# chen-bowen/instacart_next_order_recommendation

Hardware: AMD Instinct MI355X
Metric: recommend_qps_top20_49k7_catalog (higher is better)
Workload: dtype f16x3 (f32 operands split into 2 f16 planes, 3 f16 MFMAs per product, f32 accumulate; fp32-level accuracy)

## Files before the change

### instacart_next_order_recommendation_amd/csrc/encoder.hip

```cpp
#include <stdlib.h>

#include <mutex>
#include <type_traits>
#include <vector>

#include "common.h"
#include "wt_gemm.h"
#include "encoder_x3.h"

namespace icrec {

__device__ __forceinline__ int find_seq(const int32_t* __restrict__ cu, int n_seqs, int t) {
    int lo = 0, hi = n_seqs;
    while (hi - lo > 1) {
        int mid = (lo + hi) >> 1;
        if (cu[mid] <= t) lo = mid; else hi = mid;
    }
    return lo;
}

template <int H, bool SPLIT>
__device__ __forceinline__ void ln_row(float (&v)[H / 64], const float* __restrict__ g, const float* __restrict__ b,
                                       float eps, float* __restrict__ out, _Float16* __restrict__ oh,
                                       _Float16* __restrict__ ol, int lane) {
// ... 134 lines not shown
    const int tid = threadIdx.x, lane = tid & 63, wave = tid >> 6;
    const int s = blockIdx.x / heads, hd = blockIdx.x % heads;
    const int t0 = cu[s], L = cu[s + 1] - t0;
    const int nkt = (L + 31) >> 5;
    if (nkt > NKT || nkt <= nlo) return;
    const int ld = 3 * H;
    const int r = lane & 31, h = lane >> 5, qb = wave;
    const bool active = qb < nkt;
    const float* bt = nullptr;
    if constexpr (BIAS) {
        __shared__ __attribute__((aligned(16))) float Bs[ATT_BIAS_LD];
        att_bias_to_lds(Bs, bias, hd, tid, NKT * 64);
        bt = Bs + att_bias_base(qb, lane);
    }
    float4 qf[D / 8];
    {
        int qr = qb * 32 + r;
        qr = qr < L ? qr : L - 1;
        const float4* qp = reinterpret_cast<const float4*>(qkv + (size_t)(t0 + qr) * ld + hd * D);
#pragma unroll
        for (int kq = 0; kq < D / 8; ++kq) {
            const float4 a = qp[2 * kq], b = qp[2 * kq + 1];
            qf[kq] = h == 0 ? make_float4(a.x, a.z, b.x, b.z) : make_float4(a.y, a.w, b.y, b.w);
        }
    }
    const bool once = KC == NKT || nkt <= KC;
    auto stage = [&](int c0, bool with_v) {
        if (!once) __syncthreads();
        const int nk = (nkt - c0 < KC ? nkt - c0 : KC) * 32;
        for (int id = tid; id < nk * (D / 4); id += NKT * 64) {
            const int row = id / (D / 4), c = id % (D / 4);
            const int key = c0 * 32 + row, rr = key < L ? key : L - 1;
            const float* src = qkv + (size_t)(t0 + rr) * ld + hd * D + c * 4;
            const float4 kv = *reinterpret_cast<const float4*>(src + H);
            float* kp = Ks + row * LDK + (c >> 1) * 8 + (c & 1) * 2;
            *reinterpret_cast<float2*>(kp) = make_float2(kv.x, kv.z);
            *reinterpret_cast<float2*>(kp + 4) = make_float2(kv.y, kv.w);
            if (with_v) *reinterpret_cast<float4*>(Vs + row * D + c * 4) = *reinterpret_cast<const float4*>(src + 2 * H);
        }
        __syncthreads();
    };
    auto score_tile = [&](int kt, int c0) {
        f32x16 t;
#pragma unroll
        for (int e = 0; e < 16; ++e) t[e] = 0.0f;
#pragma unroll
        for (int kq = 0; kq < D / 8; ++kq) {
            const float4 kf = *reinterpret_cast<const float4*>(Ks + ((kt - c0) * 32 + r) * LDK + kq * 8 + h * 4);
            t = __builtin_amdgcn_mfma_f32_32x32x2f32(kf.x, qf[kq].x, t, 0, 0, 0);
            t = __builtin_amdgcn_mfma_f32_32x32x2f32(kf.y, qf[kq].y, t, 0, 0, 0);
            t = __builtin_amdgcn_mfma_f32_32x32x2f32(kf.z, qf[kq].z, t, 0, 0, 0);
            t = __builtin_amdgcn_mfma_f32_32x32x2f32(kf.w, qf[kq].w, t, 0, 0, 0);
        }
        const bool last = kt == nkt - 1;
#pragma unroll
        for (int e = 0; e < 16; ++e) {
            float v;
            if constexpr (BIAS) v = fmaf(t[e], scale_log2e, bt[kt * 32 + (e & 3) + 8 * (e >> 2)]);
            else v = t[e] * scale_log2e;
            if (last && kt * 32 + acc_row(e, lane) >= L) v = -INFINITY;
            t[e] = v;
        }
        return t;
    };
    f32x16 o[D / 32];
#pragma unroll
    for (int dt = 0; dt < D / 32; ++dt)
#pragma unroll
        for (int e = 0; e < 16; ++e) o[dt][e] = 0.0f;
    auto pv_tile = [&](int kt, int c0, const f32x16& p) {
#pragma unroll
        for (int e = 0; e < 16; ++e) {
            const int key = (kt - c0) * 32 + (e & 3) + 8 * (e >> 2) + 4 * h;
#pragma unroll
            for (int dt = 0; dt < D / 32; ++dt)
                o[dt] = __builtin_amdgcn_mfma_f32_32x32x2f32(p[e], Vs[key * D + 32 * dt + r], o[dt], 0, 0, 0);
        }
    };
    auto for_tiles = [&](bool with_v, auto&& f) {
#pragma unroll
        for (int c0 = 0; c0 < NKT; c0 += KC) {
            if (c0 < nkt) {
                if (!once) stage(c0, with_v);
                if (active) {
                    const int c1 = c0 + KC < nkt ? c0 + KC : nkt;
                    for (int kt = c0; kt < c1; ++kt) f(kt, c0);
                }
            }
        }
    };
    if (once) stage(0, true);
    float lsum = 0.0f;
    if constexpr (RECOMP) {
        float mx = -INFINITY;
        for_tiles(false, [&](int kt, int c0) {
            const f32x16 t = score_tile(kt, c0);
#pragma unroll
            for (int e = 0; e < 16; ++e) mx = fmaxf(mx, t[e]);
        });
        mx = fmaxf(mx, __shfl_xor(mx, 32, 64));
        for_tiles(true, [&](int kt, int c0) {
            f32x16 t = score_tile(kt, c0);
#pragma unroll
            for (int e = 0; e < 16; ++e) {
                const float p = __builtin_amdgcn_exp2f(t[e] - mx);
                t[e] = p;
                lsum = lsum + p;
            }
            pv_tile(kt, c0, t);
        });
    } else if (active) {
        f32x16 sc[NKT];
        float mx = -INFINITY;
#pragma unroll
        for (int kt = 0; kt < NKT; ++kt) {
            if (kt < nkt) {
                sc[kt] = score_tile(kt, 0);
#pragma unroll
                for (int e = 0; e < 16; ++e) mx = fmaxf(mx, sc[kt][e]);
            }
        }
        mx = fmaxf(mx, __shfl_xor(mx, 32, 64));
#pragma unroll
        for (int kt = 0; kt < NKT; ++kt) {
            if (kt < nkt) {
#pragma unroll
                for (int e = 0; e < 16; ++e) {
                    const float p = __builtin_amdgcn_exp2f(sc[kt][e] - mx);
                    sc[kt][e] = p;
                    lsum = lsum + p;
                }
            }
        }
#pragma unroll
        for (int kt = 0; kt < NKT; ++kt)
            if (kt < nkt) pv_tile(kt, 0, sc[kt]);
    }
    if (!active) return;
    lsum = join_halves(lsum, h);
    if (h == 0) Ls[wave * 32 + r] = lsum;
#pragma unroll
    for (int e = 0; e < 16; ++e) {
        const int qrow = acc_row(e, lane);
        const int tq = qb * 32 + qrow;
        if (tq < L) {
            const float l = Ls[wave * 32 + qrow];
            float* dst = ctx + (size_t)(t0 + tq) * H + hd * D + r;
#pragma unroll
            for (int dt = 0; dt < D / 32; ++dt) dst[32 * dt] = o[dt][e] / l;
        }
    }
}

__global__ __launch_bounds__(1024) void seq_order_kernel(const int32_t* __restrict__ cu, int n_seqs,
                                                         int32_t* __restrict__ order) {
    constexpr int NB = ICREC_MAX_SEQLEN / 32;
    __shared__ int hist[NB];
    const int tid = threadIdx.x;
    if (tid < NB) hist[tid] = 0;
    __syncthreads();
    auto bin = [&](int s) {
        const int L = cu[s + 1] - cu[s];
        const int nkt = (L + 31) >> 5;
        return NB - (nkt < 1 ? 1 : (nkt > NB ? NB : nkt));
    };
    for (int s0 = tid; s0 < n_seqs; s0 += 1024) atomicAdd(&hist[bin(n_seqs - 1 - s0)], 1);
    __syncthreads();
    if (tid == 0) {
        int run = 0;
        for (int b = 0; b < NB; ++b) { const int c = hist[b]; hist[b] = run; run += c; }
    }
    __syncthreads();
    for (int s0 = tid; s0 < n_seqs; s0 += 1024) {
        const int s = n_seqs - 1 - s0;
        order[atomicAdd(&hist[bin(s)], 1)] = s;
    }
}

typedef _Float16 half2v __attribute__((ext_vector_type(2)));

__device__ __forceinline__ half4 lds_read_tr(const _Float16* p) {
    typedef __fp16 fp16x4 __attribute__((__vector_size__(4 * sizeof(__fp16))));
    return __builtin_bit_cast(half4, __builtin_amdgcn_ds_read_tr16_b64_v4f16(
                                         (__attribute__((address_space(3))) fp16x4*)(reinterpret_cast<uintptr_t>(p))));
}

constexpr int att_k_swz(int D, int row) { return D == 32 ? (row >> 2) & 3 : row & 7; }
constexpr int att_x3_wgs(int D, int NKT) { return D != 32 ? 1 : NKT >= 6 ? 4 : NKT == 4 ? 3 : 1; }

template <int D, int NKT, bool BIAS = false>
__global__ __launch_bounds__(NKT * 64, att_x3_wgs(D, NKT)) void attention_x3_kernel(
    const float* __restrict__ qkv, const int32_t* __restrict__ cu, int heads, int H, float scale_log2e,
    _Float16* __restrict__ ch, _Float16* __restrict__ cl, const int32_t* __restrict__ order, int nlo, int nqb,
    const float* __restrict__ bias) {
    constexpr int KC = att_kc(D, NKT), G = D / 4;
    constexpr bool RECOMP = D == 64 || NKT >= 6;
    constexpr bool PREFETCH = D == 32, PARK = D == 32;
    static_assert(!PARK || KC == NKT, "the parked output tiles need the K planes of all NKT key tiles");
    __shared__ __attribute__((aligned(16))) _Float16 Kbuf[2 * KC * 32 * D];
    _Float16* const Kh = Kbuf;
    _Float16* const Kl = Kbuf + KC * 32 * D;
    __shared__ __attribute__((aligned(16))) _Float16 Vh[KC * 32 * D];
    __shared__ __attribute__((aligned(16))) _Float16 Vl[KC * 32 * D];
    __shared__ float Ls[NKT * 32];

    const int tid = threadIdx.x, lane = tid & 63, wave = tid >> 6;
    const int sidx = blockIdx.x / heads, hd = blockIdx.x % heads;
    const int s = order != nullptr ? order[sidx] : sidx;
    const int t0 = cu[s], L = cu[s + 1] - t0;
    const int nkt = (L + 31) >> 5;
    if (nkt > NKT || nkt <= nlo) return;
    const int ld = 3 * H;
    const int r = lane & 31, h = lane >> 5, qb = wave;
    const bool active = qb < nkt && qb < nqb;
    const float* bt = nullptr;
    if constexpr (BIAS) {
        __shared__ __attribute__((aligned(16))) float Bs[ATT_BIAS_LD];
        att_bias_to_lds(Bs, bias, hd, tid, NKT * 64);
        bt = Bs + att_bias_base(qb, lane);
    }
    half8 qh[D / 16], ql[D / 16];
    {
        int qr = qb * 32 + r;
        qr = qr < L ? qr : L - 1;
        const float* qp = qkv + (size_t)(t0 + qr) * ld + hd * D;
#pragma unroll
        for (int ks = 0; ks < D / 16; ++ks) {
            const f32x4 a = *reinterpret_cast<const f32x4*>(qp + 16 * ks + 8 * h);
            const f32x4 b = *reinterpret_cast<const f32x4*>(qp + 16 * ks + 8 * h + 4);
            half4 ah, al, bh, bl;
            split_act4(a, ah, al);
            split_act4(b, bh, bl);
            qh[ks] = half8{ah[0], ah[1], ah[2], ah[3], bh[0], bh[1], bh[2], bh[3]};
            ql[ks] = half8{al[0], al[1], al[2], al[3], bl[0], bl[1], bl[2], bl[3]};
        }
    }
    const bool once = KC == NKT || nkt <= KC;
    auto stage = [&](int c0, bool with_v) {
        if (!once) __syncthreads();
        const int nk = (nkt - c0 < KC ? nkt - c0 : KC) * 32;
        auto src_of = [&](int id) {
            const int key = c0 * 32 + id / G, rr = key < L ? key : L - 1;
            return qkv + (size_t)(t0 + rr) * ld + hd * D + (id % G) * 4;
        };
        auto put = [&](int id, const f32x4& k, const f32x4& v) {
            const int row = id / G, c = id % G;
            half4 khi, klo;
            split_act4(k, khi, klo);
            if (with_v) {
                half4 vhi, vlo;
                split_act4(v, vhi, vlo);
                *reinterpret_cast<half4*>(Vh + row * D + c * 4) = vhi;
                *reinterpret_cast<half4*>(Vl + row * D + c * 4) = vlo;
            }
            const int off = row * D + ((((c >> 1) ^ att_k_swz(D, row)) << 3) | ((c & 1) << 2));
            *reinterpret_cast<half4*>(Kh + off) = khi;
            *reinterpret_cast<half4*>(Kl + off) = klo;
        };
        if constexpr (PREFETCH) {
            constexpr int STG = KC * 32 * G / (NKT * 64);
            static_assert(KC * 32 * G % (NKT * 64) == 0, "staging: whole rounds");
            f32x4 kreg[STG], vreg[STG];
#pragma unroll
            for (int it = 0; it < STG; ++it) {
                const float* src = src_of(tid + it * NKT * 64);
                kreg[it] = *reinterpret_cast<const f32x4*>(src + H);
                if (with_v) vreg[it] = *reinterpret_cast<const f32x4*>(src + 2 * H);
            }
#pragma unroll
            for (int it = 0; it < STG; ++it)
                if (tid + it * NKT * 64 < nk * G) put(tid + it * NKT * 64, kreg[it], vreg[it]);
        } else {
            for (int id = tid; id < nk * G; id += NKT * 64) {
                const float* src = src_of(id);
                f32x4 v = {0.0f, 0.0f, 0.0f, 0.0f};
                if (with_v) v = *reinterpret_cast<const f32x4*>(src + 2 * H);
                put(id, *reinterpret_cast<const f32x4*>(src + H), v);
            }
        }
        __syncthreads();
    };
    auto score_tile = [&](int kt, int c0, bool hi_only) {
        f32x16 t;
#pragma unroll
        for (int e = 0; e < 16; ++e) t[e] = 0.0f;
        const int row = (kt - c0) * 32 + r;
#pragma unroll
        for (int ks = 0; ks < D / 16; ++ks) {
            const int off = row * D + (((2 * ks + h) ^ att_k_swz(D, row)) << 3);
            const half8 kh = *reinterpret_cast<const half8*>(Kh + off);
            const half8 kl = *reinterpret_cast<const half8*>(Kl + off);
            t = __builtin_amdgcn_mfma_f32_32x32x16_f16(kh, qh[ks], t, 0, 0, 0);
            if (hi_only) continue;
            t = __builtin_amdgcn_mfma_f32_32x32x16_f16(kh, ql[ks], t, 0, 0, 0);
            t = __builtin_amdgcn_mfma_f32_32x32x16_f16(kl, qh[ks], t, 0, 0, 0);
        }
        if (kt == nkt - 1 && kt * 32 + 32 > L) {
#pragma unroll
            for (int e = 0; e < 16; ++e)
                if (kt * 32 + acc_row(e, lane) >= L) t[e] = -INFINITY;
        }
        return t;
    };
    f32x16 o[D / 32];
#pragma unroll
    for (int dt = 0; dt < D / 32; ++dt)
#pragma unroll
        for (int e = 0; e < 16; ++e) o[dt][e] = 0.0f;
    auto pv_tile = [&](int kt, int c0, const f32x16& pt) {
#pragma unroll
        for (int ks = 0; ks < 2; ++ks) {
            half8 ph, pl;
#pragma unroll
            for (int j = 0; j < 8; j += 2) {
                half2w a, b;
                split_pair_prescaled(pt[8 * ks + j], pt[8 * ks + j + 1], a, b);
                ph[j] = a[0]; ph[j + 1] = a[1];
                pl[j] = b[0]; pl[j + 1] = b[1];
            }
            const int base = (kt - c0) * 32 + 4 * h + 16 * ks;
#pragma unroll
            for (int dt = 0; dt < D / 32; ++dt) {
                const int tr_at = (base + ((lane & 15) >> 2)) * D + 32 * dt + 16 * ((lane >> 4) & 1) + 4 * (lane & 3);
                const half4 v0h = lds_read_tr(Vh + tr_at);
                const half4 v1h = lds_read_tr(Vh + tr_at + 8 * D);
                const half4 v0l = lds_read_tr(Vl + tr_at);
                const half4 v1l = lds_read_tr(Vl + tr_at + 8 * D);
                const half8 vh = {v0h[0], v0h[1], v0h[2], v0h[3], v1h[0], v1h[1], v1h[2], v1h[3]};
                const half8 vl = {v0l[0], v0l[1], v0l[2], v0l[3], v1l[0], v1l[1], v1l[2], v1l[3]};
                o[dt] = __builtin_amdgcn_mfma_f32_32x32x16_f16(ph, vh, o[dt], 0, 0, 0);
                o[dt] = __builtin_amdgcn_mfma_f32_32x32x16_f16(ph, vl, o[dt], 0, 0, 0);
                o[dt] = __builtin_amdgcn_mfma_f32_32x32x16_f16(pl, vh, o[dt], 0, 0, 0);
            }
        }
    };
    auto for_tiles = [&](bool with_v, auto&& f) {
#pragma unroll
        for (int c0 = 0; c0 < NKT; c0 += KC) {
            if (c0 < nkt) {
                if (!once) stage(c0, with_v);
                if (active) {
#pragma unroll
                    for (int j = 0; j < KC; ++j)
                        if (c0 + j < nkt) f(c0 + j, c0);
                }
            }
        }
    };
    typedef float float2w __attribute__((ext_vector_type(2)));
    const float cs = scale_log2e * (1.0f / 256.0f);
    auto biased = [&](f32x16& t, int kt) {
#pragma unroll
        for (int e = 0; e < 16; ++e) t[e] = fmaf(t[e], cs, bt[kt * 32 + (e & 3) + 8 * (e >> 2)]);
    };
    float2w ls2 = float2w{0.0f, 0.0f};
    auto join_rows = [&]() {
        const float lrow = join_halves(ls2[0] + ls2[1], h);
        if (h == 0) Ls[wave * 32 + r] = lrow;
    };
    if (once) stage(0, true);
// ... 224 lines not shown
    __syncthreads();
    float* const ps = hs;
#pragma unroll
    for (int r = 0; r < JPT; ++r)
#pragma unroll
        for (int sl = 0; sl < S; ++sl) ps[(tid + 384 * r) * S + sl] = tanhf(acc[r][sl]);
    __syncthreads();
    if (tid < S && s0 + tid < n_seqs) {
        float logit = bc[0];
        for (int j = 0; j < H; ++j) logit = fmaf(wc[j], ps[j * S + tid], logit);
        scores[s0 + tid] = logit;
    }
}

constexpr int HID = 384;
constexpr int HID_BASE = 768;
template <class F>
static auto for_hidden(int hidden, F f) {
    return hidden == HID_BASE ? f(std::integral_constant<int, HID_BASE>{}) : f(std::integral_constant<int, HID>{});
}

struct LayerW {
    float *Wqkv, *bqkv, *Wo, *bo, *g1, *b1n, *W1, *b1, *W2, *b2, *g2, *b2n;
    _Float16 *Wqkv_p, *Wo_p, *W1_p, *W2_p;
};
struct Encoder {
    icrec_bert_cfg cfg;
    int device = 0;
    int n_cu = 256;
    int max_seqlen = 256;
    int pooling = ICREC_POOL_MEAN;
    float* att_bias = nullptr;
    float* score_head = nullptr;
    float* blob = nullptr;
    float* extra = nullptr;
    _Float16* planes = nullptr;
    float *word, *pos, *type, *eg, *eb;
    LayerW layers[64];
    bool fuse = true, side_stream = true, cls_prune = true;
    int small_m = 3584;
    int tail_m = 2560;
    struct Side {
        hipStream_t caller = nullptr, side = nullptr;
        hipEvent_t ev = nullptr;
    };
    std::mutex side_mu;
    std::vector<Side*> sides;
};

static int side_for(Encoder* e, hipStream_t caller, Encoder::Side** out) {
    std::lock_guard<std::mutex> lock(e->side_mu);
    *out = nullptr;
    for (Encoder::Side* sd : e->sides)
        if (sd->caller == caller) { *out = sd; return ICREC_OK; }
    hipStreamCaptureStatus cap = hipStreamCaptureStatusNone;
    if (caller && hipStreamIsCapturing(caller, &cap) == hipSuccess && cap != hipStreamCaptureStatusNone)
        return ICREC_OK;
    Encoder::Side* sd = new Encoder::Side();
    sd->caller = caller;
    ICREC_HIP(hipStreamCreateWithFlags(&sd->side, hipStreamNonBlocking));
    ICREC_HIP(hipEventCreateWithFlags(&sd->ev, hipEventDisableTiming));
    e->sides.push_back(sd);
    *out = sd;
    return ICREC_OK;
}

static size_t weight_count(const icrec_bert_cfg* c) {
    const size_t H = c->hidden, I = c->intermediate;
    const size_t emb = (size_t)c->vocab_size * H + (size_t)c->max_position * H + (size_t)c->type_vocab * H + 2 * H;
    const size_t per = 4 * (H * H + H) + 2 * H + (I * H + I) + (H * I + H) + 2 * H;
    return emb + per * c->layers;
}

struct EncWs {
    size_t x, xs, qkv, ctx, t1, h, total;
};
static EncWs enc_ws(const icrec_bert_cfg& c, int64_t T, bool post_only = false) {
    auto al = [](size_t b) { return (b + 255) & ~(size_t)255; };
    EncWs w;
    size_t o = 0;
    w.x = o;   o += post_only ? 0 : al((size_t)T * c.hidden * 4);
    w.xs = o;  o += al((size_t)T * c.hidden * 4);
    w.qkv = o; o += post_only ? 0 : al((size_t)T * 3 * c.hidden * 4);
    w.ctx = o; o += al((size_t)T * c.hidden * 4);
    w.t1 = o;  o += al((size_t)T * c.hidden * 4);
    w.h = o;   o += al((size_t)T * c.intermediate * 4);
    w.total = o;
    return w;
}

struct EncBufs {
    float *x, *qkv, *ctx, *t1, *h;
    _Float16 *xh, *xl, *ch, *cl, *hh, *hl;
    EncBufs(char* base, const EncWs& w, const icrec_bert_cfg& c, size_t T)
        : x(reinterpret_cast<float*>(base + w.x)), qkv(reinterpret_cast<float*>(base + w.qkv)),
          ctx(reinterpret_cast<float*>(base + w.ctx)), t1(reinterpret_cast<float*>(base + w.t1)),
          h(reinterpret_cast<float*>(base + w.h)), xh(reinterpret_cast<_Float16*>(base + w.xs)), xl(xh + T * c.hidden),
          ch(reinterpret_cast<_Float16*>(ctx)), cl(ch + T * c.hidden), hh(reinterpret_cast<_Float16*>(h)),
          hl(hh + T * c.intermediate) {}
};

static bool cls_prunes(const Encoder* e) {
    return e->pooling == ICREC_POOL_CLS && e->cls_prune && e->cfg.gemm_mode == ICREC_GEMM_F16X3;
}

typedef TileCfg<2, 2, 2, 2> GemmBig;
constexpr long long SMALL_M_MAX = 1 << 20;

static int env_knob(const char* name, int fallback, long long hi) {
    const char* s = getenv(name);
    if (!s) return fallback;
    char* end = nullptr;
    const long long v = strtoll(s, &end, 10);
    if (end == s) return fallback;
    return (int)(v < 0 ? 0 : v > hi ? hi : v);
}

template <bool GELU>
static void launch_linear(const float* A, int M, int K, const float* W, int N, const float* bias, float* out,
                          hipStream_t st) {
    const int mt = (M + GemmBig::BM - 1) / GemmBig::BM, nt = (N + GemmBig::BN - 1) / GemmBig::BN;
    hipLaunchKernelGGL((linear_kernel<GemmBig, GELU>), dim3(mt * nt), dim3(GemmBig::THREADS), 0, st, A, M, K, W, N,
                       bias, out, nt);
}

template <int EPI>
static void launch_wt_linear(const _Float16* Xh, const _Float16* Xl, int T, int K, const _Float16* Wp, int N,
                             const float* bias, float* out, _Float16* oh, _Float16* ol, hipStream_t st, bool small) {
    if (small) {
        if constexpr (EPI == 0 || EPI == 2) {
            const int nbn = N / 64;
            auto kern = K % 256 == 0 && K >= 1024 ? wt_linear_half_kernel<EPI, 8> : wt_linear_half_kernel<EPI, 6>;
            hipLaunchKernelGGL(kern, dim3(((T + 31) / 32) * nbn), dim3(256), 0, st, Xh, Xl, T, K, Wp, N, bias, out,
                               (const _Float16*)oh, (const _Float16*)ol, nbn);
        } else {
            const int nbn = N / 128;
            hipLaunchKernelGGL((wt_linear_kernel<1, 1, 4, EPI>), dim3(((T + 31) / 32) * nbn), dim3(256), 0, st, Xh, Xl, T, K,
                               Wp, N, bias, out, oh, ol, nbn);
        }
    } else {
        const int nbn = N / 384;
        auto kern = wt_linear_kernel<3, 2, 1, EPI>;
        if constexpr (EPI == 2) kern = for_hidden(N, [](auto h) { return wt_linear_kernel<3, 2, 1, 2, h()>; });
        hipLaunchKernelGGL(kern, dim3(((T + 63) / 64) * nbn), dim3(256), 0, st, Xh, Xl, T, K, Wp, N, bias, out, oh, ol,
                           nbn);
    }
}

enum AttBucket { ATT_9_16, ATT_1, ATT_2, ATT_3_4, ATT_5_6, ATT_7_8, ATT_5_8, ATT_N };
constexpr int ATT_LO[ATT_N] = {9, 1, 2, 3, 5, 7, 5}, ATT_HI[ATT_N] = {16, 1, 2, 4, 6, 8, 8};

template <bool X3>
static void launch_attention(unsigned mask, const icrec_bert_cfg& c, const EncBufs& b, const int32_t* cu, int n_seqs,
                             int max_seqlen, const int32_t* order, const float* bias, hipStream_t st,
                             bool block0_only = false) {
    const int nkt_max = (max_seqlen + 31) / 32;
    const int dh = c.hidden / c.heads;
    const bool single = n_seqs == 1, split_5_8 = X3 && !single && dh == 32;
    const float sl2e = (1.0f / sqrtf((float)dh)) * 1.44269504088896340736f;
    for (int k = 0; k < ATT_N; ++k) {
        if (!(mask >> k & 1) || (split_5_8 ? k == ATT_5_8 : k == ATT_5_6 || k == ATT_7_8) || nkt_max < ATT_LO[k] ||
            (single && nkt_max > ATT_HI[k]))
            continue;
        const dim3 grid(n_seqs * c.heads), block(ATT_HI[k] * 64);
        if constexpr (X3) {
#define ICREC_ATT_ROW(K, D, B) {K<D, 16, B>, K<D, 1, B>, K<D, 2, B>, K<D, 4, B>, D == 32 ? K<32, 6, B> : nullptr, D == 32 ? K<32, 8, B> : nullptr, K<D, 8, B>}
            static const decltype(&attention_x3_kernel<32, 1>) kern[2][2][ATT_N] = {
                {ICREC_ATT_ROW(attention_x3_kernel, 32, false), ICREC_ATT_ROW(attention_x3_kernel, 64, false)},
                {ICREC_ATT_ROW(attention_x3_kernel, 32, true), ICREC_ATT_ROW(attention_x3_kernel, 64, true)}};
#undef ICREC_ATT_ROW
            hipLaunchKernelGGL(kern[bias != nullptr][dh == 64][k], grid, block, 0, st, b.qkv, cu, c.heads, c.hidden, sl2e,
                               b.ch, b.cl, order, ATT_LO[k] - 1, block0_only ? 1 : ATT_HI[k], bias);
        } else {
#define ICREC_ATT_ROW(D, B) {attention_kernel<D, 16, B>, attention_kernel<D, 1, B>, attention_kernel<D, 2, B>, attention_kernel<D, 4, B>, nullptr, nullptr, attention_kernel<D, 8, B>}
            static const decltype(&attention_kernel<32, 1>) kern[2][2][ATT_N] = {
                {ICREC_ATT_ROW(32, false), ICREC_ATT_ROW(64, false)}, {ICREC_ATT_ROW(32, true), ICREC_ATT_ROW(64, true)}};
#undef ICREC_ATT_ROW
            hipLaunchKernelGGL(kern[bias != nullptr][dh == 64][k], grid, block, 0, st, b.qkv, cu, c.heads, c.hidden, sl2e,
                               b.ctx, ATT_LO[k] - 1, bias);
        }
    }
}

}

using namespace icrec;

extern "C" {

size_t icrec_encoder_weight_count(const icrec_bert_cfg* cfg) { return cfg ? weight_count(cfg) : 0; }

int icrec_encoder_create(const float* weights_host, size_t n_floats, const icrec_bert_cfg* cfg, int device,
                         icrec_encoder** out) {
    ICREC_REQUIRE(weights_host && cfg && out, "icrec_encoder_create: NULL argument");
    ICREC_REQUIRE((cfg->hidden == HID && cfg->heads * 32 == HID) || (cfg->hidden == HID_BASE && cfg->heads * 64 == HID_BASE),
                  "icrec_encoder_create: (hidden, heads) must be (384, 12) or (768, 12): head_dim 32 at hidden 384, head_dim 64 "
                  "at hidden 768 (got hidden=%d, heads=%d)", cfg->hidden, cfg->heads);
    ICREC_REQUIRE(cfg->intermediate >= 384 && cfg->intermediate % 384 == 0, "icrec_encoder_create: intermediate size must be a multiple of 384 (got %d)", cfg->intermediate);
    ICREC_REQUIRE(cfg->layers >= 1 && cfg->layers <= 64, "icrec_encoder_create: layers must be in [1,64]");
    ICREC_REQUIRE(cfg->vocab_size >= 1 && cfg->max_position >= 1 && cfg->type_vocab >= 1, "icrec_encoder_create: bad vocab/position sizes");
    ICREC_REQUIRE(cfg->n_normalize >= 0 && cfg->n_normalize <= 4, "icrec_encoder_create: n_normalize must be in [0,4]");
    ICREC_REQUIRE(cfg->gemm_mode == ICREC_GEMM_F32 || cfg->gemm_mode == ICREC_GEMM_F16X3, "icrec_encoder_create: unknown gemm_mode %d", cfg->gemm_mode);
    ICREC_REQUIRE(n_floats == weight_count(cfg), "icrec_encoder_create: weight blob has %zu floats, expected %zu", n_floats, weight_count(cfg));
    ICREC_HIP(hipSetDevice(device));
    hipDeviceProp_t prop;
    ICREC_HIP(hipGetDeviceProperties(&prop, device));
    if (strncmp(prop.gcnArchName, "gfx950", 6) != 0) {
        set_error("icrec_encoder_create: device %d is %s, this library is built for gfx950 only", device, prop.gcnArchName);
        return ICREC_ENODEV;
    }
    Encoder* e = new Encoder();
    e->cfg = *cfg;
    e->device = device;
    e->n_cu = prop.multiProcessorCount > 0 ? prop.multiProcessorCount : 256;
    e->max_seqlen = cfg->max_position < 256 ? cfg->max_position : 256;
    {
        const char* fuse_env = getenv("ICREC_FUSE");
        const char* side_env = getenv("ICREC_SIDE_STREAM");
        e->fuse = !(fuse_env && fuse_env[0] == '0');
        e->small_m = env_knob("ICREC_SMALL_M", e->small_m, SMALL_M_MAX);
        e->tail_m = env_knob("ICREC_TAIL_M", e->tail_m, 64LL * e->n_cu - 1);
        e->side_stream = !(side_env && side_env[0] == '0');
        const char* prune_env = getenv("ICREC_CLS_PRUNE");
        e->cls_prune = !(prune_env && prune_env[0] == '0');
    }
    const size_t H = cfg->hidden, I = cfg->intermediate;
    const size_t mat_per_layer = 3 * H * H + H * H + I * H + H * I;
    const bool x3 = cfg->gemm_mode == ICREC_GEMM_F16X3;
    if (hipMalloc(&e->blob, n_floats * 4) != hipSuccess ||
        hipMalloc(&e->extra, (size_t)cfg->layers * (3 * H * H + 3 * H) * 4) != hipSuccess ||
        (x3 && hipMalloc(&e->planes, (size_t)cfg->layers * mat_per_layer * 2 * sizeof(_Float16)) != hipSuccess)) {
        set_error("icrec_encoder_create: hipMalloc failed");
        if (e->blob) (void)hipFree(e->blob);
        if (e->extra) (void)hipFree(e->extra);
        delete e;
        return ICREC_ENOMEM;
    }
    ICREC_HIP(hipMemcpy(e->blob, weights_host, n_floats * 4, hipMemcpyHostToDevice));
    float* p = e->blob;
    e->word = p; p += (size_t)cfg->vocab_size * H;
    e->pos = p;  p += (size_t)cfg->max_position * H;
    e->type = p; p += (size_t)cfg->type_vocab * H;
    e->eg = p;   p += H;
    e->eb = p;   p += H;
    float* x = e->extra;
    _Float16* pl = e->planes;
    auto pack = [&](const float* w, int N, int K, _Float16*& out) {
        out = pl;
        pl += (size_t)2 * N * K;
        hipLaunchKernelGGL(pack_weights_kernel, dim3(1024), dim3(256), 0, 0, w, N, K, out);
    };
    for (int l = 0; l < cfg->layers; ++l) {
        LayerW& L = e->layers[l];
        L.Wqkv = x; x += 3 * H * H;
        L.bqkv = x; x += 3 * H;
        for (int part = 0; part < 3; ++part) {
            ICREC_HIP(hipMemcpy(L.Wqkv + part * H * H, p, H * H * 4, hipMemcpyDeviceToDevice)); p += H * H;
            ICREC_HIP(hipMemcpy(L.bqkv + part * H, p, H * 4, hipMemcpyDeviceToDevice)); p += H;
        }
        L.Wo = p; p += H * H; L.bo = p; p += H;
        L.g1 = p; p += H; L.b1n = p; p += H;
        L.W1 = p; p += I * H; L.b1 = p; p += I;
        L.W2 = p; p += H * I; L.b2 = p; p += H;
        L.g2 = p; p += H; L.b2n = p; p += H;
        if (x3) {
            pack(L.Wqkv, (int)(3 * H), (int)H, L.Wqkv_p);
            pack(L.Wo, (int)H, (int)H, L.Wo_p);
            pack(L.W1, (int)I, (int)H, L.W1_p);
            pack(L.W2, (int)H, (int)I, L.W2_p);
        }
    }
    ICREC_HIP(hipGetLastError());
    ICREC_HIP(hipDeviceSynchronize());
    *out = reinterpret_cast<icrec_encoder*>(e);
    return ICREC_OK;
}

int icrec_encoder_destroy(icrec_encoder* h) {
    Encoder* e = reinterpret_cast<Encoder*>(h);
    if (!e) return ICREC_OK;
    (void)hipSetDevice(e->device);
    (void)hipFree(e->blob);
    (void)hipFree(e->extra);
    if (e->planes) (void)hipFree(e->planes);
    if (e->att_bias) (void)hipFree(e->att_bias);
    if (e->score_head) (void)hipFree(e->score_head);
    for (Encoder::Side* sd : e->sides) {
        (void)hipStreamSynchronize(sd->side);
        (void)hipStreamDestroy(sd->side);
        (void)hipEventDestroy(sd->ev);
        delete sd;
    }
    delete e;
    return ICREC_OK;
}

int icrec_encoder_set_max_seqlen(icrec_encoder* h, int32_t max_seqlen) {
    Encoder* e = reinterpret_cast<Encoder*>(h);
    ICREC_REQUIRE(e, "icrec_encoder_set_max_seqlen: NULL encoder");
    const int hi = e->cfg.max_position < ICREC_MAX_SEQLEN ? e->cfg.max_position : ICREC_MAX_SEQLEN;
    ICREC_REQUIRE(max_seqlen >= 1 && max_seqlen <= hi, "icrec_encoder_set_max_seqlen: max_seqlen must be in [1, %d] (got %d)", hi, max_seqlen);
    e->max_seqlen = max_seqlen;
    return ICREC_OK;
}

int icrec_encoder_set_pooling(icrec_encoder* h, int32_t mode) {
    Encoder* e = reinterpret_cast<Encoder*>(h);
    ICREC_REQUIRE(e, "icrec_encoder_set_pooling: NULL encoder");
    ICREC_REQUIRE(mode == ICREC_POOL_MEAN || mode == ICREC_POOL_CLS, "icrec_encoder_set_pooling: mode must be ICREC_POOL_MEAN (0) or ICREC_POOL_CLS (1) (got %d)", mode);
    e->pooling = mode;
    return ICREC_OK;
}

int32_t icrec_encoder_pooling(const icrec_encoder* h) {
    const Encoder* e = reinterpret_cast<const Encoder*>(h);
    return e ? e->pooling : -1;
}

int icrec_encoder_set_attention_bias(icrec_encoder* h, const float* bias_host, int32_t heads) {
    Encoder* e = reinterpret_cast<Encoder*>(h);
    ICREC_REQUIRE(e, "icrec_encoder_set_attention_bias: NULL encoder");
    ICREC_HIP(hipSetDevice(e->device));
    if (!bias_host) {
        if (e->att_bias) ICREC_HIP(hipFree(e->att_bias));
        e->att_bias = nullptr;
// ... 56 lines not shown
    float* dev = e->score_head;
    if (!dev && hipMalloc(&dev, host.size() * 4) != hipSuccess) {
        set_error("icrec_encoder_set_score_head: hipMalloc failed");
        return ICREC_ENOMEM;
    }
    const hipError_t err = hipMemcpy(dev, host.data(), host.size() * 4, hipMemcpyHostToDevice);
    if (err != hipSuccess && !e->score_head) (void)hipFree(dev);
    ICREC_HIP(err);
    e->score_head = dev;
    return ICREC_OK;
}

int32_t icrec_encoder_has_score_head(const icrec_encoder* h) {
    const Encoder* e = reinterpret_cast<const Encoder*>(h);
    return e ? (e->score_head != nullptr) : -1;
}

static size_t workspace_bytes(const Encoder* e, int64_t T, int n_seqs) {
    return enc_ws(e->cfg, T).total + (cls_prunes(e) ? enc_ws(e->cfg, n_seqs, true).total : 0);
}

size_t icrec_encode_workspace_bytes(const icrec_encoder* h, int64_t total_tokens, int32_t n_seqs) {
    const Encoder* e = reinterpret_cast<const Encoder*>(h);
    if (!e || total_tokens < 1 || n_seqs < 1) return 0;
    return workspace_bytes(e, total_tokens, n_seqs);
}

static int batch_tail(const Encoder* e, int T) {
    const int round_tokens = 64 * e->n_cu;
    return T > round_tokens && T % round_tokens <= e->tail_m ? T % round_tokens : 0;
}

int icrec_encode_batch_split(const icrec_encoder* h, int64_t total_tokens, int64_t* main_tokens, int64_t* tail_tokens) {
    const Encoder* e = reinterpret_cast<const Encoder*>(h);
    ICREC_REQUIRE(e && main_tokens && tail_tokens && total_tokens >= 1 && total_tokens < (1ll << 31), "icrec_encode_batch_split: bad argument");
    *tail_tokens = batch_tail(e, (int)total_tokens);
    *main_tokens = total_tokens - *tail_tokens;
    return ICREC_OK;
}

static const int32_t* embed(const Encoder* e, const EncBufs& b, const int32_t* ids_dev, const int32_t* cu_dev,
                            const int32_t* seg_b_dev, int n_seqs, int T, hipStream_t st) {
    const icrec_bert_cfg& c = e->cfg;
    const bool x3 = c.gemm_mode == ICREC_GEMM_F16X3;
    int32_t* order = nullptr;
    if (x3 && n_seqs >= 64 && e->fuse) {
        order = reinterpret_cast<int32_t*>(b.x);
        hipLaunchKernelGGL(seq_order_kernel, dim3(1), dim3(1024), 0, st, cu_dev, n_seqs, order);
    }
    auto kern =
        for_hidden(c.hidden, [x3](auto h) { return x3 ? embed_ln_kernel<h(), true> : embed_ln_kernel<h(), false>; });
    if (seg_b_dev)
        kern = for_hidden(c.hidden, [x3](auto h) { return x3 ? embed_ln_kernel<h(), true, true> : embed_ln_kernel<h(), false, true>; });
    hipLaunchKernelGGL(kern, dim3((T + 3) / 4), dim3(256), 0, st, ids_dev, cu_dev, n_seqs, T, e->word, e->pos, e->type, e->eg, e->eb, c.ln_eps, c.vocab_size,
                       c.max_position, b.x, b.xh, b.xl, seg_b_dev);
    return order;
}

static hipError_t link(const Encoder::Side* sd, hipStream_t from, hipStream_t to) {
    const hipError_t err = hipEventRecord(sd->ev, from);
    return err != hipSuccess ? err : hipStreamWaitEvent(to, sd->ev, 0);
}

struct Range {
    int r0, n;
    hipStream_t st;
    bool small;
    bool layer;
    bool fold;
    Range(const Encoder* e, int r0, int n, hipStream_t st)
        : r0(r0), n(n), st(st), small(n <= e->small_m), layer(e->fuse && !small && e->cfg.hidden == HID),
          fold(e->fuse && small && e->cfg.hidden == HID) {}
    bool launches_qkv(int l) const { return l == 0 || !layer; }
    bool ffn_ln_to_next(int l, int layers) const { return fold && l + 1 < layers; }
};

static int encode_x3(Encoder* e, const EncBufs& b, const EncBufs* cls, const int32_t* cu_dev, int n_seqs, int T,
                     int max_seqlen, const int32_t* order, hipStream_t st) {
    const icrec_bert_cfg& c = e->cfg;
    const int H = c.hidden, I = c.intermediate;
    const auto ln_wt = for_hidden(H, [](auto h) { return ln_wt_kernel<h()>; });
    const bool split_att = H == HID && e->side_stream && n_seqs >= 64 && max_seqlen > 128;
    const int T_tail = batch_tail(e, T), T_main = T - T_tail;
    Encoder::Side* sd = nullptr;
    if (e->side_stream && (T_tail || split_att))
        if (int rc_ = side_for(e, st, &sd)) return rc_;
    const Range main(e, 0, T_main, st), tail(e, T_main, T_tail, sd ? sd->side : st);
    const bool tail_on_side = T_tail && sd;
    if (main.layer || tail.layer) {
        if (int rc_ = ensure_dynamic_lds(reinterpret_cast<const void*>(qkv_resident_kernel), QKVR_LDS)) return rc_;
        if (int rc_ = ensure_dynamic_lds(reinterpret_cast<const void*>(ffn_fused2_kernel), FFN2_LDS)) return rc_;
    }

    auto qkv_stage = [&](const Range& r, int l) {
        const LayerW& L = e->layers[l];
        _Float16 *const xhr = b.xh + (size_t)r.r0 * H, *const xlr = b.xl + (size_t)r.r0 * H;
        float* const qkvr = b.qkv + (size_t)r.r0 * 3 * H;
        if (r.layer) {
            hipLaunchKernelGGL(qkv_resident_kernel, dim3((r.n + 63) / 64), dim3(512), QKVR_LDS, r.st, xhr, xlr, r.n,
                               L.Wqkv_p, L.bqkv, qkvr, 3 * H);
        } else if (l > 0 && r.ffn_ln_to_next(l - 1, c.layers)) {
            const LayerW& Lp = e->layers[l - 1];
            const int nbn = 3 * H / 64;
            hipLaunchKernelGGL((wt_linear_lnin_kernel<0>), dim3(((r.n + 31) / 32) * nbn), dim3(256), 0, r.st,
                               (const float*)(b.t1 + (size_t)r.r0 * H), r.n, Lp.g2, Lp.b2n, c.ln_eps, xhr, xlr, L.Wqkv_p,
                               3 * H, L.bqkv, qkvr, (_Float16*)nullptr, (_Float16*)nullptr, nbn);
        } else {
            launch_wt_linear<0>(xhr, xlr, r.n, H, L.Wqkv_p, 3 * H, L.bqkv, qkvr, nullptr, nullptr, r.st, r.small);
        }
    };
    auto post_stage = [&](const Range& r, int l, const EncBufs& b) {
        const LayerW& L = e->layers[l];
        float* const t1r = b.t1 + (size_t)r.r0 * H;
        _Float16 *const xhr = b.xh + (size_t)r.r0 * H, *const xlr = b.xl + (size_t)r.r0 * H;
        const _Float16 *const chr = b.ch + (size_t)r.r0 * H, *const clr = b.cl + (size_t)r.r0 * H;
        if (r.layer) {
            ScopedTimer tm(T_FFN_UP, r.st);
            const bool next_qkv = l + 1 < c.layers;
            const LayerW& Ln = e->layers[next_qkv ? l + 1 : l];
            hipLaunchKernelGGL(ffn_fused2_kernel, dim3((r.n + 63) / 64), dim3(512), FFN2_LDS, r.st, xhr, xlr, r.n, I,
                               L.W1_p, L.b1, L.W2_p, L.b2, L.g2, L.b2n, c.ln_eps, chr, clr, L.Wo_p, L.bo, L.g1, L.b1n,
                               next_qkv ? (const _Float16*)Ln.Wqkv_p : (const _Float16*)nullptr, (const float*)Ln.bqkv,
                               b.qkv + (size_t)r.r0 * 3 * H, 3 * H);
            return;
        }
        _Float16 *const hhr = b.hh + (size_t)r.r0 * I, *const hlr = b.hl + (size_t)r.r0 * I;
        launch_wt_linear<2>(chr, clr, r.n, H, L.Wo_p, H, L.bo, t1r, xhr, xlr, r.st, r.small);
        if (r.fold) {
            const int nbn = I / 64;
            hipLaunchKernelGGL((wt_linear_lnin_kernel<1>), dim3(((r.n + 31) / 32) * nbn), dim3(256), 0, r.st,
                               (const float*)t1r, r.n, L.g1, L.b1n, c.ln_eps, xhr, xlr, L.W1_p, I, L.b1, (float*)nullptr,
                               hhr, hlr, nbn);
        } else {
            hipLaunchKernelGGL(ln_wt, dim3((r.n + 15) / 16), dim3(256), 0, r.st, t1r, r.n, L.g1, L.b1n, c.ln_eps,
                               xhr, xlr);
            ScopedTimer tm(r.small ? T_NSLOTS - 1 : T_FFN_UP, r.st);
            launch_wt_linear<1>(xhr, xlr, r.n, H, L.W1_p, I, L.b1, nullptr, hhr, hlr, r.st, r.small);
        }
        launch_wt_linear<2>(hhr, hlr, r.n, I, L.W2_p, H, L.b2, t1r, xhr, xlr, r.st, r.small);
        if (!r.ffn_ln_to_next(l, c.layers))
            hipLaunchKernelGGL(ln_wt, dim3((r.n + 15) / 16), dim3(256), 0, r.st, t1r, r.n, L.g2, L.b2n, c.ln_eps,
                               xhr, xlr);
    };

    if (tail_on_side) ICREC_HIP(link(sd, st, sd->side));
    for (int l = 0; l < c.layers; ++l) {
        const bool pruned = cls && l == c.layers - 1;
        if (T_tail && tail.launches_qkv(l)) qkv_stage(tail, l);
        if (main.launches_qkv(l)) qkv_stage(main, l);
        if (tail_on_side) ICREC_HIP(link(sd, sd->side, st));
        if (split_att && sd) {
            ICREC_HIP(link(sd, st, sd->side));
            const unsigned side_buckets = 1u << ATT_1 | 1u << ATT_2 | 1u << ATT_3_4 | 1u << ATT_7_8;
            launch_attention<true>(1u << ATT_9_16, c, b, cu_dev, n_seqs, max_seqlen, order, e->att_bias, st, pruned);
            launch_attention<true>(side_buckets, c, b, cu_dev, n_seqs, max_seqlen, order, e->att_bias, sd->side, pruned);
            launch_attention<true>(1u << ATT_5_6, c, b, cu_dev, n_seqs, max_seqlen, order, e->att_bias, st, pruned);
            ICREC_HIP(link(sd, sd->side, st));
        } else {
            launch_attention<true>(~0u, c, b, cu_dev, n_seqs, max_seqlen, order, e->att_bias, st, pruned);
        }
        if (pruned) {
            hipLaunchKernelGGL(gather_cls_rows_kernel, dim3((n_seqs * (H / 8) + 255) / 256), dim3(256), 0, st, b.ch, b.cl,
                               b.xh, b.xl, cu_dev, n_seqs, H / 8, cls->ch, cls->cl, cls->xh, cls->xl);
            Range rows(e, 0, n_seqs, st);
            rows.layer = false;
            post_stage(rows, l, *cls);
            return ICREC_OK;
        }
        if (tail_on_side) ICREC_HIP(link(sd, st, sd->side));
        if (T_tail) post_stage(tail, l, b);
        post_stage(main, l, b);
    }
    if (tail_on_side) ICREC_HIP(link(sd, sd->side, st));
    return ICREC_OK;
}

static int encode_f32(const Encoder* e, const EncBufs& b, const int32_t* cu_dev, int n_seqs, int T, int max_seqlen,
                      hipStream_t st) {
    const icrec_bert_cfg& c = e->cfg;
    const int H = c.hidden, I = c.intermediate, rows_grid = (T + 3) / 4;
    const auto add_ln = for_hidden(H, [](auto h) { return add_ln_kernel<h()>; });
    for (int l = 0; l < c.layers; ++l) {
        const LayerW& L = e->layers[l];
        launch_linear<false>(b.x, T, H, L.Wqkv, 3 * H, L.bqkv, b.qkv, st);
        launch_attention<false>(~0u, c, b, cu_dev, n_seqs, max_seqlen, nullptr, e->att_bias, st);
        launch_linear<false>(b.ctx, T, H, L.Wo, H, L.bo, b.t1, st);
        hipLaunchKernelGGL(add_ln, dim3(rows_grid), dim3(256), 0, st, b.t1, b.x, T, L.g1, L.b1n,
                           c.ln_eps, b.xh, b.xl);
        {
            ScopedTimer tm(T_FFN_UP, st);
            launch_linear<true>(b.x, T, H, L.W1, I, L.b1, b.h, st);
        }
        launch_linear<false>(b.h, T, I, L.W2, H, L.b2, b.t1, st);
        hipLaunchKernelGGL(add_ln, dim3(rows_grid), dim3(256), 0, st, b.t1, b.x, T, L.g2, L.b2n,
                           c.ln_eps, b.xh, b.xl);
    }
    return ICREC_OK;
}

int icrec_encode(icrec_encoder* h, const int32_t* ids_dev, const int32_t* cu_dev, int32_t n_seqs, int64_t T64,
                 int32_t max_seqlen, float* out_dev, void* ws, size_t ws_bytes, void* stream) {
    return icrec_encode_ex(h, ids_dev, cu_dev, n_seqs, T64, max_seqlen, out_dev, nullptr, ws, ws_bytes, stream);
}

int icrec_encode_ex(icrec_encoder* h, const int32_t* ids_dev, const int32_t* cu_dev, int32_t n_seqs, int64_t T64,
                    int32_t max_seqlen, float* out_dev, float* tokens_out_dev, void* ws, size_t ws_bytes,
                    void* stream) {
    Encoder* e = reinterpret_cast<Encoder*>(h);
    ICREC_REQUIRE(e && ids_dev && cu_dev && out_dev, "icrec_encode: NULL argument");
    ICREC_REQUIRE((reinterpret_cast<uintptr_t>(tokens_out_dev) & 15) == 0, "icrec_encode_ex: tokens_out_dev must be 16-byte aligned");
    ICREC_REQUIRE(n_seqs >= 1 && T64 >= n_seqs && T64 < (1ll << 31), "icrec_encode: bad n_seqs/total_tokens (%d, %lld)", n_seqs, (long long)T64);
    ICREC_REQUIRE(max_seqlen >= 1 && max_seqlen <= e->max_seqlen, "icrec_encode: max_seqlen must be in [1, %d] (got %d)", e->max_seqlen, max_seqlen);
    const int T = (int)T64;
    const EncWs w = enc_ws(e->cfg, T);
    const size_t need = workspace_bytes(e, T, n_seqs);
    if (!ws || ws_bytes < need) {
        set_error("icrec_encode: workspace too small (%zu < %zu)", ws_bytes, need);
        return ICREC_ENOMEM;
    }
    ICREC_HIP(hipSetDevice(e->device));
    hipStream_t st = (hipStream_t)stream;
    ScopedTimer whole(T_ENCODE, st);
    char* base = reinterpret_cast<char*>(ws);
    const icrec_bert_cfg& c = e->cfg;
    const int H = c.hidden;
    const bool x3 = c.gemm_mode == ICREC_GEMM_F16X3;
    const EncBufs b(base, w, c, T);
    const bool pruned = cls_prunes(e) && !tokens_out_dev && n_seqs < T;
    const EncBufs cls(base + w.total, enc_ws(c, n_seqs, true), c, n_seqs);
    const int32_t* order = embed(e, b, ids_dev, cu_dev, nullptr, n_seqs, T, st);
    if (int rc_ = x3 ? encode_x3(e, b, pruned ? &cls : nullptr, cu_dev, n_seqs, T, max_seqlen, order, st)
                     : encode_f32(e, b, cu_dev, n_seqs, T, max_seqlen, st))
        return rc_;
    const auto pool =
        for_hidden(H, [x3](auto h) { return x3 ? pool_norm_kernel<h(), true> : pool_norm_kernel<h(), false>; });
    const EncBufs& last = pruned ? cls : b;
    const int pool_rows = e->pooling != ICREC_POOL_CLS ? POOL_ROWS_MEAN : pruned ? POOL_ROWS_CLS_COMPACT : POOL_ROWS_CLS;
    hipLaunchKernelGGL(pool, dim3(n_seqs), dim3(H), 0, st, last.x, last.xh, last.xl, cu_dev, c.n_normalize, out_dev,
                       pool_rows);
    if (tokens_out_dev) {
        const size_t n4 = (size_t)T * H / 4;
        hipLaunchKernelGGL(x3 ? tokens_out_kernel<true> : tokens_out_kernel<false>, dim3((unsigned)((n4 + 255) / 256)),
                           dim3(256), 0, st, b.x, b.xh, b.xl, n4, tokens_out_dev);
    }
    ICREC_HIP(hipGetLastError());
    return ICREC_OK;
}

static bool score_prunes(const Encoder* e) { return e->cls_prune && e->cfg.gemm_mode == ICREC_GEMM_F16X3; }

size_t icrec_score_pairs_workspace_bytes(const icrec_encoder* h, int64_t total_tokens, int32_t n_seqs) {
    const Encoder* e = reinterpret_cast<const Encoder*>(h);
    if (!e || total_tokens < 1 || n_seqs < 1) return 0;
    return enc_ws(e->cfg, total_tokens).total + (score_prunes(e) ? enc_ws(e->cfg, n_seqs, true).total : 0);
}

int icrec_score_pairs(icrec_encoder* h, const int32_t* ids_dev, const int32_t* cu_dev, const int32_t* seg_b_dev,
                      int32_t n_seqs, int64_t T64, int32_t max_seqlen, float* scores_out_dev, void* ws, size_t ws_bytes,
                      void* stream) {
    Encoder* e = reinterpret_cast<Encoder*>(h);
    ICREC_REQUIRE(e && ids_dev && cu_dev && seg_b_dev && scores_out_dev, "icrec_score_pairs: NULL argument");
    ICREC_REQUIRE(e->score_head, "icrec_score_pairs: the encoder has no score head (icrec_encoder_set_score_head)");
    ICREC_REQUIRE(n_seqs >= 1 && T64 >= n_seqs && T64 < (1ll << 31), "icrec_score_pairs: bad n_seqs/total_tokens (%d, %lld)", n_seqs, (long long)T64);
    ICREC_REQUIRE(max_seqlen >= 1 && max_seqlen <= e->max_seqlen, "icrec_score_pairs: max_seqlen must be in [1, %d] (got %d)", e->max_seqlen, max_seqlen);
    const int T = (int)T64;
    const size_t need = icrec_score_pairs_workspace_bytes(h, T, n_seqs);
    if (!ws || ws_bytes < need) {
        set_error("icrec_score_pairs: workspace too small (%zu < %zu)", ws_bytes, need);
        return ICREC_ENOMEM;
    }
    ICREC_HIP(hipSetDevice(e->device));
    hipStream_t st = (hipStream_t)stream;
    char* base = reinterpret_cast<char*>(ws);
    const icrec_bert_cfg& c = e->cfg;
    const int H = c.hidden;
    const bool x3 = c.gemm_mode == ICREC_GEMM_F16X3;
    const EncWs w = enc_ws(c, T);
    const EncBufs b(base, w, c, T);
    const bool pruned = score_prunes(e) && n_seqs < T;
    const EncBufs cls(base + w.total, enc_ws(c, n_seqs, true), c, n_seqs);
    const int32_t* order = embed(e, b, ids_dev, cu_dev, seg_b_dev, n_seqs, T, st);
    if (int rc_ = x3 ? encode_x3(e, b, pruned ? &cls : nullptr, cu_dev, n_seqs, T, max_seqlen, order, st)
                     : encode_f32(e, b, cu_dev, n_seqs, T, max_seqlen, st))
        return rc_;
    const EncBufs& last = pruned ? cls : b;
    const float *const wpt = e->score_head, *const bp = wpt + (size_t)H * H, *const wc = bp + H, *const bc = wc + H;
    const auto kern =
        for_hidden(H, [x3](auto h) { return x3 ? score_head_kernel<h(), true> : score_head_kernel<h(), false>; });
    const int per_wg = H == HID_BASE ? HEAD_SEQS<HID_BASE> : HEAD_SEQS<HID>;
    hipLaunchKernelGGL(kern, dim3((n_seqs + per_wg - 1) / per_wg), dim3(384), 0, st, last.x, last.xh, last.xl, cu_dev,
                       n_seqs, pruned, wpt, bp, wc, bc, scores_out_dev);
    ICREC_HIP(hipGetLastError());
    return ICREC_OK;
}

}
```

Before: 110,800.

## Publish length-bin bounds from seq_order and skip empty attention workgroups

The sequence-ordering kernel now writes the prefix-sum bin boundaries after the order array. Each attention kernel offsets its block index by the start of its key-tile bucket and exits early past the bucket end. The host also shrinks each grid using a bound derived from total tokens. For head dim 32, the 1- and 2-tile buckets are folded into the 3-4 tile launch, which removes launches and idle workgroups but runs short sequences with larger blocks. The order buffer must now have room for the extra bin entries.

```diff
diff --git a/instacart_next_order_recommendation_amd/csrc/encoder.hip b/instacart_next_order_recommendation_amd/csrc/encoder.hip
--- a/instacart_next_order_recommendation_amd/csrc/encoder.hip
+++ b/instacart_next_order_recommendation_amd/csrc/encoder.hip
@@ -310,9 +310,11 @@
     }
 }
 
+constexpr int ATT_ORDER_BINS = ICREC_MAX_SEQLEN / 32;
+
 __global__ __launch_bounds__(1024) void seq_order_kernel(const int32_t* __restrict__ cu, int n_seqs,
                                                          int32_t* __restrict__ order) {
-    constexpr int NB = ICREC_MAX_SEQLEN / 32;
+    constexpr int NB = ATT_ORDER_BINS;
     __shared__ int hist[NB];
     const int tid = threadIdx.x;
     if (tid < NB) hist[tid] = 0;
@@ -326,7 +328,8 @@
     __syncthreads();
     if (tid == 0) {
         int run = 0;
-        for (int b = 0; b < NB; ++b) { const int c = hist[b]; hist[b] = run; run += c; }
+        for (int b = 0; b < NB; ++b) { const int c = hist[b]; hist[b] = run; order[n_seqs + b] = run; run += c; }
+        order[n_seqs + NB] = run;
     }
     __syncthreads();
     for (int s0 = tid; s0 < n_seqs; s0 += 1024) {
@@ -349,12 +352,13 @@
 template <int D, int NKT, bool BIAS = false>
 __global__ __launch_bounds__(NKT * 64, att_x3_wgs(D, NKT)) void attention_x3_kernel(
     const float* __restrict__ qkv, const int32_t* __restrict__ cu, int heads, int H, float scale_log2e,
-    _Float16* __restrict__ ch, _Float16* __restrict__ cl, const int32_t* __restrict__ order, int nlo, int nqb,
-    const float* __restrict__ bias) {
+    _Float16* __restrict__ ch, _Float16* __restrict__ cl, const int32_t* __restrict__ order, int n_seqs, int nlo,
+    int nqb, const float* __restrict__ bias) {
     constexpr int KC = att_kc(D, NKT), G = D / 4;
     constexpr bool RECOMP = D == 64 || NKT >= 6;
     constexpr bool PREFETCH = D == 32, PARK = D == 32;
     static_assert(!PARK || KC == NKT, "the parked output tiles need the K planes of all NKT key tiles");
+    static_assert(NKT <= ATT_ORDER_BINS, "seq_order_kernel publishes a bound per key-tile count up to ATT_ORDER_BINS");
     __shared__ __attribute__((aligned(16))) _Float16 Kbuf[2 * KC * 32 * D];
     _Float16* const Kh = Kbuf;
     _Float16* const Kl = Kbuf + KC * 32 * D;
@@ -363,7 +367,13 @@
     __shared__ float Ls[NKT * 32];
 
     const int tid = threadIdx.x, lane = tid & 63, wave = tid >> 6;
-    const int sidx = blockIdx.x / heads, hd = blockIdx.x % heads;
+    int sidx = blockIdx.x / heads;
+    const int hd = blockIdx.x % heads;
+    if (order != nullptr) {
+        const int32_t* const bound = order + n_seqs;
+        sidx += bound[ATT_ORDER_BINS - NKT];
+        if (sidx >= bound[ATT_ORDER_BINS - nlo]) return;
+    }
     const int s = order != nullptr ? order[sidx] : sidx;
     const int t0 = cu[s], L = cu[s + 1] - t0;
     const int nkt = (L + 31) >> 5;
@@ -894,17 +904,22 @@
 
 template <bool X3>
 static void launch_attention(unsigned mask, const icrec_bert_cfg& c, const EncBufs& b, const int32_t* cu, int n_seqs,
-                             int max_seqlen, const int32_t* order, const float* bias, hipStream_t st,
+                             int T, int max_seqlen, const int32_t* order, const float* bias, hipStream_t st,
                              bool block0_only = false) {
     const int nkt_max = (max_seqlen + 31) / 32;
     const int dh = c.hidden / c.heads;
     const bool single = n_seqs == 1, split_5_8 = X3 && !single && dh == 32;
+    const bool fold = X3 && order != nullptr && dh == 32 && nkt_max >= ATT_LO[ATT_3_4];
     const float sl2e = (1.0f / sqrtf((float)dh)) * 1.44269504088896340736f;
     for (int k = 0; k < ATT_N; ++k) {
         if (!(mask >> k & 1) || (split_5_8 ? k == ATT_5_8 : k == ATT_5_6 || k == ATT_7_8) || nkt_max < ATT_LO[k] ||
-            (single && nkt_max > ATT_HI[k]))
+            (single && nkt_max > ATT_HI[k]) || (fold && (k == ATT_1 || k == ATT_2)))
             continue;
-        const dim3 grid(n_seqs * c.heads), block(ATT_HI[k] * 64);
+        const int lo = fold && k == ATT_3_4 ? 1 : ATT_LO[k];
+        int n_wg_seqs = n_seqs;
+        if (order != nullptr) n_wg_seqs = std::min(n_seqs, T / (32 * (lo - 1) + 1));
+        if (n_wg_seqs == 0) continue;
+        const dim3 grid(n_wg_seqs * c.heads), block(ATT_HI[k] * 64);
         if constexpr (X3) {
 #define ICREC_ATT_ROW(K, D, B) {K<D, 16, B>, K<D, 1, B>, K<D, 2, B>, K<D, 4, B>, D == 32 ? K<32, 6, B> : nullptr, D == 32 ? K<32, 8, B> : nullptr, K<D, 8, B>}
             static const decltype(&attention_x3_kernel<32, 1>) kern[2][2][ATT_N] = {
@@ -912,7 +927,7 @@
                 {ICREC_ATT_ROW(attention_x3_kernel, 32, true), ICREC_ATT_ROW(attention_x3_kernel, 64, true)}};
 #undef ICREC_ATT_ROW
             hipLaunchKernelGGL(kern[bias != nullptr][dh == 64][k], grid, block, 0, st, b.qkv, cu, c.heads, c.hidden, sl2e,
-                               b.ch, b.cl, order, ATT_LO[k] - 1, block0_only ? 1 : ATT_HI[k], bias);
+                               b.ch, b.cl, order, n_seqs, lo - 1, block0_only ? 1 : ATT_HI[k], bias);
         } else {
 #define ICREC_ATT_ROW(D, B) {attention_kernel<D, 16, B>, attention_kernel<D, 1, B>, attention_kernel<D, 2, B>, attention_kernel<D, 4, B>, nullptr, nullptr, attention_kernel<D, 8, B>}
             static const decltype(&attention_kernel<32, 1>) kern[2][2][ATT_N] = {
@@ -1275,12 +1290,12 @@
         if (split_att && sd) {
             ICREC_HIP(link(sd, st, sd->side));
             const unsigned side_buckets = 1u << ATT_1 | 1u << ATT_2 | 1u << ATT_3_4 | 1u << ATT_7_8;
-            launch_attention<true>(1u << ATT_9_16, c, b, cu_dev, n_seqs, max_seqlen, order, e->att_bias, st, pruned);
-            launch_attention<true>(side_buckets, c, b, cu_dev, n_seqs, max_seqlen, order, e->att_bias, sd->side, pruned);
-            launch_attention<true>(1u << ATT_5_6, c, b, cu_dev, n_seqs, max_seqlen, order, e->att_bias, st, pruned);
+            launch_attention<true>(1u << ATT_9_16, c, b, cu_dev, n_seqs, T, max_seqlen, order, e->att_bias, st, pruned);
+            launch_attention<true>(side_buckets, c, b, cu_dev, n_seqs, T, max_seqlen, order, e->att_bias, sd->side, pruned);
+            launch_attention<true>(1u << ATT_5_6, c, b, cu_dev, n_seqs, T, max_seqlen, order, e->att_bias, st, pruned);
             ICREC_HIP(link(sd, sd->side, st));
         } else {
-            launch_attention<true>(~0u, c, b, cu_dev, n_seqs, max_seqlen, order, e->att_bias, st, pruned);
+            launch_attention<true>(~0u, c, b, cu_dev, n_seqs, T, max_seqlen, order, e->att_bias, st, pruned);
         }
         if (pruned) {
             hipLaunchKernelGGL(gather_cls_rows_kernel, dim3((n_seqs * (H / 8) + 255) / 256), dim3(256), 0, st, b.ch, b.cl,
@@ -1306,7 +1321,7 @@
     for (int l = 0; l < c.layers; ++l) {
         const LayerW& L = e->layers[l];
         launch_linear<false>(b.x, T, H, L.Wqkv, 3 * H, L.bqkv, b.qkv, st);
-        launch_attention<false>(~0u, c, b, cu_dev, n_seqs, max_seqlen, nullptr, e->att_bias, st);
+        launch_attention<false>(~0u, c, b, cu_dev, n_seqs, T, max_seqlen, nullptr, e->att_bias, st);
         launch_linear<false>(b.ctx, T, H, L.Wo, H, L.bo, b.t1, st);
         hipLaunchKernelGGL(add_ln, dim3(rows_grid), dim3(256), 0, st, b.t1, b.x, T, L.g1, L.b1n,
                            c.ln_eps, b.xh, b.xl);
```

Measured after the change: 111,400, median of 6. About the same (+0.5%).
